# mynameisfiber/baton

Measured on NVIDIA H100. Metric: federated local samples/sec (whole box), ResNet-18 FedAvg, synthetic non-IID 32x32 shards, higher is better.
Workload: dtype bf16

## Files before the change

baton_b200/csrc/bindings.cpp:

```cpp
#include <ATen/cuda/CUDAContext.h>
#include <c10/cuda/CUDAGuard.h>
#include <torch/extension.h>

#include <optional>
#include <vector>

#include "launch.h"

namespace {

inline cudaStream_t cur_stream() { return at::cuda::getCurrentCUDAStream().stream(); }
inline void check(int rc, const char* what) {
  TORCH_CHECK(rc == 0, "baton_b200::", what, " failed with code ", rc,
              rc > 0 ? std::string(" (") + cudaGetErrorString(static_cast<cudaError_t>(rc)) + ")" : std::string());
}
inline const void* cptr(const at::Tensor& t) { return t.data_ptr(); }
inline void* ptr(at::Tensor& t) { return t.data_ptr(); }
template <class T>
inline T* opt_ptr(const std::optional<at::Tensor>& t) {
  return (t.has_value() && t->defined()) ? reinterpret_cast<T*>(t->data_ptr()) : nullptr;
}
#define CHECK_CUDA(x) TORCH_CHECK((x).is_cuda(), #x " must be a CUDA tensor")

inline const float* prox_anchor(const std::optional<at::Tensor>& anchor, int64_t numel, const at::Tensor& hyper) {
// ... 220 lines not shown
  return true;
}
bool conv_halo(const at::Tensor& src, const at::Tensor& w, at::Tensor out, int64_t stride, bool dgrad, int64_t mc,
               const std::optional<at::Tensor>& col_stats) {
  CHECK_CUDA(src); CHECK_CUDA(w); CHECK_CUDA(out);
  TORCH_CHECK(src.scalar_type() == at::kBFloat16 && w.scalar_type() == at::kBFloat16 && out.scalar_type() == at::kBFloat16 &&
              src.dim() == 4 && src.is_contiguous() && w.is_contiguous() && out.is_contiguous());
  TORCH_CHECK(stride == 1 || stride == 2, "conv_halo: stride 1 or 2");
  const int64_t c = src.size(3);
  const int64_t rows = src.size(0) * ((src.size(1) - 1) / stride + 1) * ((src.size(2) - 1) / stride + 1);
  TORCH_CHECK(rows > 0 && out.numel() % rows == 0, "conv_halo: out must hold [N*Ho*Wo, Nout] elements");
  const int64_t nout = out.numel() / rows;
  TORCH_CHECK(w.numel() == (dgrad ? c * 9 * nout : nout * 9 * c), "conv_halo: w must be [Cout, 9*Cin]");
  TORCH_CHECK(dgrad ? !col_stats.has_value()
                    : (!col_stats.has_value() || (col_stats->scalar_type() == at::kFloat && col_stats->numel() >= 2 * nout)),
              "conv_halo: col_stats is a [2 Cout] fp32 buffer of the forward");
  const c10::cuda::CUDAGuard guard(src.device());
  const int rc = b200_conv_halo(cptr(src), cptr(w), ptr(out), static_cast<int>(src.size(0)), static_cast<int>(src.size(1)),
                                static_cast<int>(src.size(2)), static_cast<int>(c), static_cast<int>(nout),
                                static_cast<int>(stride), dgrad ? 1 : 0, static_cast<int>(mc), opt_ptr<float>(col_stats),
                                cur_stream());
  if (rc == -2) return false;
  check(rc, "conv_halo");
  return true;
}
bool conv_igemm_dgrad_s2(const at::Tensor& dy, const at::Tensor& w, at::Tensor dx, int64_t kh, int64_t kw,
                         const std::vector<int64_t>& ntaps, const std::vector<int64_t>& taps, int64_t force_bn) {
  CHECK_CUDA(dy); CHECK_CUDA(w); CHECK_CUDA(dx);
  TORCH_CHECK(dy.scalar_type() == at::kBFloat16 && w.scalar_type() == at::kBFloat16 && dx.scalar_type() == at::kBFloat16 &&
              dy.dim() == 4 && dx.dim() == 4 && dy.is_contiguous() && w.is_contiguous() && dx.is_contiguous());
  TORCH_CHECK(ntaps.size() == 4 && taps.size() == 16, "conv_igemm_dgrad_s2: 4 classes x 4 taps");
  int nt[4], tw[16];
  for (int i = 0; i < 4; ++i) nt[i] = static_cast<int>(ntaps[i]);
  for (int i = 0; i < 16; ++i) tw[i] = static_cast<int>(taps[i]);
  const c10::cuda::CUDAGuard guard(dy.device());
  const int rc = b200_conv_igemm_dgrad_s2(cptr(dy), cptr(w), ptr(dx), static_cast<int>(dx.size(0)),
                                          static_cast<int>(dx.size(1)), static_cast<int>(dx.size(2)),
                                          static_cast<int>(dx.size(3)), static_cast<int>(dy.size(3)), static_cast<int>(kh),
                                          static_cast<int>(kw), static_cast<int>(dy.size(1)), static_cast<int>(dy.size(2)),
                                          nt, tw, static_cast<int>(force_bn), cur_stream());
  if (rc == -2) return false;
  check(rc, "conv_igemm_dgrad_s2");
  return true;
}
bool conv_igemm_wgrad(const at::Tensor& dy, const at::Tensor& x, at::Tensor dw, int64_t cout, int64_t kh, int64_t kw,
                      int64_t stride, int64_t pad, int64_t ho, int64_t wo, int64_t split_k, int64_t force_bn,
// ... 818 lines not shown
  const int in32 = pred.scalar_type() == at::kFloat;
  const int out32 = dpred.has_value() && dpred->defined() && dpred->scalar_type() == at::kFloat;
  check(b200_mse(pred.data_ptr(), in32, target.data_ptr<float>(), opt_ptr<void>(dpred), out32,
                 loss_acc.data_ptr<float>(), pred.numel(), static_cast<float>(grad_scale), cur_stream()),
        "mse");
}

}

PYBIND11_MODULE(TORCH_EXTENSION_NAME, m) {
  m.doc() = "baton_b200 sm_90a kernels";
  m.attr("MAX_RANKS") = B200_MAX_RANKS;
  m.def("gemm", &gemm);
  m.def("trace_set", &trace_set);
  m.def("attention_fwd", &attention_fwd);
  m.def("attention_bwd", &attention_bwd);
  m.def("bn_bwd_cluster", &bn_bwd_cluster);
  m.def("im2col_tma_probe", &im2col_tma_probe);
  m.def("conv_igemm_fwd", &conv_igemm_fwd);
  m.def("conv_igemm_wgrad", &conv_igemm_wgrad);
  m.def("conv_igemm_dgrad", &conv_igemm_dgrad);
  m.def("conv_igemm_dgrad_s2", &conv_igemm_dgrad_s2);
  m.def("conv_halo", &conv_halo);
  m.def("gemm_batched", &gemm_batched);
  m.def("gemm_fp8", &gemm_fp8);
  m.def("quant_mx_rows", &quant_mx_rows);
  m.def("quant_mx_cols", &quant_mx_cols);
  m.def("fused_sgd", &fused_sgd);
  m.def("fused_sgd_segments", &fused_sgd_segments);
  m.def("weighted_sum", &weighted_sum);
  m.def("fold_client", &fold_client);
  m.def("scaffold_corr", &scaffold_corr);
  m.def("scaffold_dc", &scaffold_dc);
  m.def("cast", &cast);
  m.def("gather_rows", &gather_rows);
  m.def("colsum", &colsum);
  m.def("add_bf16", &add_bf16);
  m.def("relu_bwd", &relu_bwd);
  m.def("gelu", &gelu);
  m.def("gelu_bwd", &gelu_bwd);
  m.def("pad_rows", &pad_rows);
  m.def("embedding_bwd", &embedding_bwd);
  m.def("fedavg_allreduce", &fedavg_allreduce);
  m.def("fedavg_allreduce_robust", &fedavg_allreduce_robust);
  m.def("fedavg_allreduce_krum", &fedavg_allreduce_krum);
  m.attr("KRUM_MAX_CTAS") = B200_KRUM_MAX_CTAS;
// ... 36 lines not shown
```

baton_b200/csrc/gemm_wgmma.cu:

```cuda
#define B200_TU_TAG 1
#include "ptx.cuh"
#include "epilogue.cuh"
#include "launch.h"
#include "pdl.cuh"
#include "sgd.cuh"

namespace b200 {

constexpr int BM = 128;
constexpr int BK = 64;
constexpr int WG_K = 16;
constexpr int GEMM_THREADS = 384;
constexpr int CONSUMER_WARPS = 8;
constexpr int CONSUMER_THREADS = 32 * CONSUMER_WARPS;
constexpr int MAX_STAGES = 8;
constexpr int S2_MAX_TAPS = 4;

struct GemmParams {
  int M, N, K;
  void* D;
  long long ldd;
  const float* bias;
  int out_fp32;
  int act;
// ... 339 lines not shown
  return w;
}
__device__ __forceinline__ int s2_dx_row(const GemmParams& p, int cls, int m) {
  if (m >= p.M) return -1;
  const int hw = p.conv_ho * p.conv_wo;
  const int n = m / hw, r = m - n * hw;
  const int i = r / p.conv_wo, j = r - i * p.conv_wo;
  const int h = 2 * i + (cls >> 1), w = 2 * j + (cls & 1);
  return (h < p.conv_h && w < p.conv_w) ? (n * p.conv_h + h) * p.conv_w + w : -1;
}
template <int BN>
__device__ __forceinline__ void s2_load_ktile(const CUtensorMap* tmA, const CUtensorMap* tmB, const GemmParams& p,
                                              uint8_t* sa, uint8_t* sb, uint64_t* bar, int cls, int kt, int m0, int n0) {
  const int cblocks = p.conv_cin >> 6;
  const int slot = kt / cblocks, cb = kt - slot * cblocks;
  const int tw = s2_tap(p, cls, slot);
  const int q0 = m0 % p.conv_wo, t0 = m0 / p.conv_wo;
  tma_load_im2col_4d(sa, tmA, bar, cb * 64, q0, t0 % p.conv_ho, t0 / p.conv_ho, (tw >> 24) & 0xff, (tw >> 16) & 0xff);
  const int wcol = (tw & 0xffff) * p.conv_ncol + n0;
#pragma unroll
  for (int j = 0; j < BN / 64; ++j) tma_load_2d(sb + j * 8192, tmB, bar, wcol + j * 64, cb * 64);
}

template <int BN, int STAGES, int CONV = 0, bool SGD = false, bool AFFINE = false, bool PROX = false, bool SCAF = false,
          bool ADAM = false>
__global__ void __launch_bounds__(GEMM_THREADS, 1)
gemm_bf16_fixed_kernel(const __grid_constant__ CUtensorMap tmA, const __grid_constant__ CUtensorMap tmB,
                         const GemmParams p) {
  using L = SmemLayout<BN>;
  static_assert(STAGES * L::STAGE_BYTES >= L::PART_BYTES, "the drained ring must hold the fp32 accumulator tile");
  extern __shared__ __align__(1024) uint8_t smem_raw[];
  uint8_t* smem = reinterpret_cast<uint8_t*>((reinterpret_cast<uintptr_t>(smem_raw) + 1023) & ~uintptr_t(1023));
  uint64_t* full_bar = reinterpret_cast<uint64_t*>(smem + STAGES * L::STAGE_BYTES);
  uint64_t* empty_bar = full_bar + STAGES;
  float* cstat = reinterpret_cast<float*>(empty_bar + STAGES);

  griddep_launch_dependents();
  const int warp = threadIdx.x >> 5;
  int m0 = blockIdx.y * BM;
  const int cls = CONV == 4 ? s2_class(p, m0) : 0;
  const int n0 = blockIdx.x * BN;
  const int k_tiles_total = CONV == 4 ? s2_ntaps(p, cls) * (p.conv_cin >> 6) : (p.K + BK - 1) / BK;
  const int bz_outer = p.batched ? static_cast<int>(blockIdx.z) / p.batch_inner : 0;
  const int bz_inner = p.batched ? static_cast<int>(blockIdx.z) % p.batch_inner : 0;
  const int kt_begin = p.batched ? 0 : blockIdx.z * p.k_tiles_per_split;
  int kt_end = kt_begin + p.k_tiles_per_split;
  if (kt_end > k_tiles_total) kt_end = k_tiles_total;
  const int num_kt = kt_end - kt_begin;

  if (warp == 0 && elect_one()) {
    tma_prefetch_desc(&tmA);
    tma_prefetch_desc(&tmB);
    for (int s = 0; s < STAGES; ++s) {
      mbar_init(&full_bar[s], 1);
      mbar_init(&empty_bar[s], CONSUMER_WARPS);
    }
    fence_barrier_init();
  }
  __syncthreads();
  griddep_wait();

  if (warp == 0) {
    if (elect_one()) {
      if (p.tile_flags != nullptr) {
        const int rows_here = (p.N - n0) < BN ? (p.N - n0) : BN;
        const uint32_t need = p.flag_epoch_ptr != nullptr ? *reinterpret_cast<const volatile uint32_t*>(p.flag_epoch_ptr)
                                                          : p.flag_epoch;
        wait_arrival_flags(p.tile_flags, p.flag_elem_off + static_cast<long long>(n0) * p.ldb,
                           p.flag_elem_off + static_cast<long long>(n0 + rows_here) * p.ldb - 1, p.flag_tile_elems, need);
        if (p.flag_bias_off >= 0)
          wait_arrival_flags(p.tile_flags, p.flag_bias_off + n0, p.flag_bias_off + n0 + rows_here - 1,
                             p.flag_tile_elems, need);
        fence_proxy_async_all();
      }
      TRACE_POINT();
      for (int i = 0; i < num_kt; ++i) {
        const int s = i % STAGES;
        const uint32_t ph = (i / STAGES) & 1;
        mbar_wait(&empty_bar[s], ph ^ 1);
        uint8_t* sa = smem + s * L::STAGE_BYTES;
        uint8_t* sb = sa + L::A_BYTES;
        const int k0 = (kt_begin + i) * BK;
        if constexpr (CONV == 2) {
          const int live = (p.N - n0 + 63) / 64 < BN / 64 ? (p.N - n0 + 63) / 64 : BN / 64;
          mbar_expect_tx(&full_bar[s], L::A_BYTES + live * 8192);
        } else {
          mbar_expect_tx(&full_bar[s], L::STAGE_BYTES);
        }
        if (p.batched) {
          if (!p.a_mn) {
            tma_load_4d(sa, &tmA, &full_bar[s], k0, m0, bz_inner, bz_outer);
          } else {
#pragma unroll
            for (int j = 0; j < BM / 64; ++j)
              tma_load_4d(sa + j * 8192, &tmA, &full_bar[s], m0 + j * 64, k0, bz_inner, bz_outer);
          }
          if (!p.b_mn) {
            tma_load_4d(sb, &tmB, &full_bar[s], k0, n0, bz_inner, bz_outer);
          } else {
#pragma unroll
            for (int j = 0; j < BN / 64; ++j)
              tma_load_4d(sb + j * 8192, &tmB, &full_bar[s], n0 + j * 64, k0, bz_inner, bz_outer);
          }
        } else if constexpr (CONV == 4) {
          s2_load_ktile<BN>(&tmA, &tmB, p, sa, sb, &full_bar[s], cls, kt_begin + i, m0, n0);
        } else {
        if constexpr (CONV == 1 || CONV == 3) {
          const int kt = kt_begin + i;
          const int cblocks = p.conv_cin >> 6;
          const int tap = kt / cblocks, cb = kt - tap * cblocks;
          const int fr = tap / p.conv_kw, fs = tap - fr * p.conv_kw;
          const int q0 = m0 % p.conv_wo, t0 = m0 / p.conv_wo;
          tma_load_im2col_4d(sa, &tmA, &full_bar[s], cb * 64, q0 * p.conv_stride - p.conv_pad,
                             (t0 % p.conv_ho) * p.conv_stride - p.conv_pad, t0 / p.conv_ho, fs, fr);
        } else if (!p.a_mn) {
          tma_load_2d(sa, &tmA, &full_bar[s], k0, m0);
        } else {
#pragma unroll
          for (int j = 0; j < BM / 64; ++j)
            tma_load_2d(sa + j * 8192, &tmA, &full_bar[s], m0 + j * 64, k0);
        }
        if constexpr (CONV == 2) {
          const int q0 = k0 % p.conv_wo, t0 = k0 / p.conv_wo;
          const int w0 = q0 * p.conv_stride - p.conv_pad, h0 = (t0 % p.conv_ho) * p.conv_stride - p.conv_pad;
          const int img = t0 / p.conv_ho;
#pragma unroll
          for (int j = 0; j < BN / 64; ++j) {
            const int col = n0 + j * 64;
// ... 96 lines not shown
        } else {
          _Pragma("unroll") for (int j = 0; j < 32; ++j) if (col0 + j < p.N) d[j] = v[j];
        }
      } else {
        __nv_bfloat16* d = reinterpret_cast<__nv_bfloat16*>(drow) + col0;
        if (full && vec_ok) {
#pragma unroll
          for (int j = 0; j < 32; j += 8) {
            uint4 o;
            o.x = pack_bf16x2(v[j], v[j + 1]);
            o.y = pack_bf16x2(v[j + 2], v[j + 3]);
            o.z = pack_bf16x2(v[j + 4], v[j + 5]);
            o.w = pack_bf16x2(v[j + 6], v[j + 7]);
            *reinterpret_cast<uint4*>(d + j) = o;
          }
        } else {
          _Pragma("unroll") for (int j = 0; j < 32; ++j) if (col0 + j < p.N) d[j] = __float2bfloat16_rn(v[j]);
        }
      }
    }
    if (threadIdx.x == 128) TRACE_POINT();
    if (want_stats) {
      named_bar_sync(1, CONSUMER_THREADS);
      for (int i = threadIdx.x - 128; i < 2 * BN; i += CONSUMER_THREADS) {
        const int col = i < BN ? i : i - BN;
        if (n0 + col < p.N)
          atomicAdd(p.col_stats + (i < BN ? 0 : p.N) + n0 + col,
                    cstat[i] + cstat[2 * BN + i] + cstat[4 * BN + i] + cstat[6 * BN + i]);
      }
    }
  }
}


constexpr int EPI_PITCH = 144;
constexpr int EPI_WARP_BYTES = 32 * EPI_PITCH;

template <int BN>
__device__ __forceinline__ void epilogue_tile(const GemmParams& p, const float* acc_tile, int q, int half, int m0,
                                              int n0, uint8_t* stage, bool vec_ok, size_t d_off = 0) {
  using L = SmemLayout<BN>;
  const int lane = static_cast<int>(lane_id());
  const int row = m0 + q * 32 + lane;
  const float* arow = acc_tile + (q * 32 + lane) * L::PART_PITCH;
  const int elt = p.out_fp32 ? 4 : 2;
  const bool fast = vec_ok && !p.atomic_out && (p.N % 8 == 0);
  if (!fast) {
#pragma unroll 1
    for (int c = half * 32; c < BN; c += 64) {
      uint32_t r[32];
      acc_ld_row32(arow + c, r);
// ... 151 lines not shown
    }
  }
}


template <int BN, bool CLUSTER, int CONV = 0, bool AFFINE = false>
__global__ void __launch_bounds__(GEMM_THREADS, 1)
gemm_bf16_splitk_kernel(const __grid_constant__ CUtensorMap tmA, const __grid_constant__ CUtensorMap tmB,
                        const GemmParams p) {
  using L = SmemLayout<BN>;
  extern __shared__ __align__(1024) uint8_t smem_raw[];
  uint8_t* smem = reinterpret_cast<uint8_t*>((reinterpret_cast<uintptr_t>(smem_raw) + 1023) & ~uintptr_t(1023));
  const int STAGES = p.stages;
  const int ring_bytes = STAGES * L::STAGE_BYTES;
  const int data_bytes = L::PART_BYTES > ring_bytes ? L::PART_BYTES : ring_bytes;
  uint64_t* full_bar = reinterpret_cast<uint64_t*>(smem + data_bytes);
  uint64_t* empty_bar = full_bar + MAX_STAGES;
  float* cstat = reinterpret_cast<float*>(empty_bar + MAX_STAGES);

  griddep_launch_dependents();
  const int warp = threadIdx.x >> 5;
  const int m0 = blockIdx.y * BM;
  const int n0 = blockIdx.x * BN;
  const int k_tiles_total = (p.K + BK - 1) / BK;
  const int kt_begin = blockIdx.z * p.k_tiles_per_split;
  int kt_end = kt_begin + p.k_tiles_per_split;
  if (kt_end > k_tiles_total) kt_end = k_tiles_total;
  const int num_kt = kt_end - kt_begin;

  if (warp == 0 && elect_one()) {
    tma_prefetch_desc(&tmA);
    tma_prefetch_desc(&tmB);
    for (int s = 0; s < STAGES; ++s) {
      mbar_init(&full_bar[s], 1);
      mbar_init(&empty_bar[s], CONSUMER_WARPS);
    }
    fence_barrier_init();
  }
  __syncthreads();
  griddep_wait();

  if (warp == 0) {
    if (elect_one()) {
      if (p.tile_flags != nullptr) {
        const int rows_here = (p.N - n0) < BN ? (p.N - n0) : BN;
        const uint32_t need = p.flag_epoch_ptr != nullptr ? *reinterpret_cast<const volatile uint32_t*>(p.flag_epoch_ptr)
                                                          : p.flag_epoch;
        wait_arrival_flags(p.tile_flags, p.flag_elem_off + static_cast<long long>(n0) * p.ldb,
                           p.flag_elem_off + static_cast<long long>(n0 + rows_here) * p.ldb - 1, p.flag_tile_elems, need);
        if (p.flag_bias_off >= 0)
          wait_arrival_flags(p.tile_flags, p.flag_bias_off + n0, p.flag_bias_off + n0 + rows_here - 1,
                             p.flag_tile_elems, need);
        fence_proxy_async_all();
      }
      int s = 0;
      uint32_t ph = 0;
      for (int i = 0; i < num_kt; ++i) {
        mbar_wait(&empty_bar[s], ph ^ 1);
        uint8_t* sa = smem + s * L::STAGE_BYTES;
        uint8_t* sb = sa + L::A_BYTES;
        const int k0 = (kt_begin + i) * BK;
        mbar_expect_tx(&full_bar[s], L::STAGE_BYTES);
        if constexpr (CONV == 1 || CONV == 3) {
          const int kt = kt_begin + i;
          const int cblocks = p.conv_cin >> 6;
          const int tap = kt / cblocks, cb = kt - tap * cblocks;
          const int fr = tap / p.conv_kw, fs = tap - fr * p.conv_kw;
          const int q0 = m0 % p.conv_wo, t0 = m0 / p.conv_wo;
          tma_load_im2col_4d(sa, &tmA, &full_bar[s], cb * 64, q0 * p.conv_stride - p.conv_pad,
                             (t0 % p.conv_ho) * p.conv_stride - p.conv_pad, t0 / p.conv_ho, fs, fr);
        } else if (!p.a_mn) {
          tma_load_2d(sa, &tmA, &full_bar[s], k0, m0);
        } else {
#pragma unroll
          for (int j = 0; j < BM / 64; ++j)
            tma_load_2d(sa + j * 8192, &tmA, &full_bar[s], m0 + j * 64, k0);
        }
        if constexpr (CONV == 3) {
          const int kt = kt_begin + i;
          const int cblocks = p.conv_cin >> 6;
          const int tap = kt / cblocks, cb = kt - tap * cblocks;
          const int wcol = (p.conv_taps - 1 - tap) * p.conv_ncol + n0;
#pragma unroll
          for (int j = 0; j < BN / 64; ++j) tma_load_2d(sb + j * 8192, &tmB, &full_bar[s], wcol + j * 64, cb * 64);
        } else if (!p.b_mn) {
          tma_load_2d(sb, &tmB, &full_bar[s], k0, n0);
        } else {
#pragma unroll
          for (int j = 0; j < BN / 64; ++j) tma_load_2d(sb + j * 8192, &tmB, &full_bar[s], n0 + j * 64, k0);
        }
        if (++s == STAGES) { s = 0; ph ^= 1; }
      }
    }
  } else if (warp >= 4) {
    const int ew = warp - 4;
    float acc[BN / 2];
    int s = 0;
    uint32_t ph = 0;
    consume_ktiles<BN>(acc, smem, STAGES, full_bar, empty_bar, s, ph, num_kt, p.a_mn, p.b_mn, ew >> 2);
    named_bar_sync(1, CONSUMER_THREADS);
    float* part = reinterpret_cast<float*>(smem);
// ... 52 lines not shown
            cq[j] = fmaf(rnd, rnd, cq[j]);
          }
        }
        if (row < p.M && col0 < p.N) store_row_chunk<8, AFFINE>(p, row, col0, v, vec_ok);
      }
      if (want_stats) {
#pragma unroll
        for (int j = 0; j < 8; ++j) {
#pragma unroll
          for (int o = CG; o < 32; o <<= 1) {
            cs[j] += __shfl_xor_sync(0xffffffffu, cs[j], o);
            cq[j] += __shfl_xor_sync(0xffffffffu, cq[j], o);
          }
        }
        const int wq = t >> 5, ln = t & 31;
        if (ln < CG) {
#pragma unroll
          for (int j = 0; j < 8; ++j) {
            cstat[wq * 2 * BN + ln * 8 + j] = cs[j];
            cstat[wq * 2 * BN + BN + ln * 8 + j] = cq[j];
          }
        }
        named_bar_sync(2, 128);
        for (int i = t; i < 2 * BN; i += 128) {
          const int col = i < BN ? i : i - BN;
          if (n0 + col < p.N) {
            const float v = cstat[i] + cstat[2 * BN + i] + cstat[4 * BN + i] + cstat[6 * BN + i];
            atomicAdd(p.col_stats + (i < BN ? 0 : p.N) + n0 + col, v);
          }
        }
      }
    }
    cluster_sync_all();
  }
}


typedef CUresult (*EncodeTiledFn)(CUtensorMap*, CUtensorMapDataType, cuuint32_t, void*, const cuuint64_t*,
                                  const cuuint64_t*, const cuuint32_t*, const cuuint32_t*, CUtensorMapInterleave,
                                  CUtensorMapSwizzle, CUtensorMapL2promotion, CUtensorMapFloatOOBfill);

static EncodeTiledFn get_encode_fn() {
  static thread_local bool ctx_bound = false;
  if (!ctx_bound) {
    cudaFree(nullptr);
    ctx_bound = true;
  }
  static EncodeTiledFn fn = nullptr;
  if (fn == nullptr) {
    void* ptr = nullptr;
    cudaDriverEntryPointQueryResult qres;
// ... 443 lines not shown
  }
  if (max_taps == 0) return -2;
  const int bn = clamp_bn(force_bn > 0 ? force_bn : (Cin > 64 ? 128 : 64));
  CUtensorMap ta, tb;
  int rc = b200_encode_map_im2col_bf16(&ta, dy, N, Ho, Wo, Cout, 1, 1, 1, 0, 64, BM);
  if (rc) return rc;
  rc = make_map(&tb, w, Cout, static_cast<long long>(KH) * KW * Cin, static_cast<long long>(KH) * KW * Cin, 64, BK);
  if (rc) return rc;
  const int k_tiles = max_taps * (Cout / 64);
  p.M = static_cast<int>(M); p.N = Cin; p.K = k_tiles * BK; p.D = dx; p.ldd = Cin; p.bias = nullptr; p.out_fp32 = 0;
  p.act = 0; p.a_mn = 0; p.b_mn = 1; p.k_tiles_per_split = k_tiles; p.cluster_k = 1; p.atomic_out = 0;
  p.col_stats = nullptr;
  p.tile_flags = nullptr; p.flag_epoch = 0; p.alpha = 1.0f; p.flag_elem_off = 0; p.flag_tile_elems = 0;
  p.ldb = static_cast<long long>(KH) * KW * Cin;
  p.flag_bias_off = -1; p.flag_epoch_ptr = nullptr;
  p.batched = 0; p.batch_inner = 1; p.batch_count = 1; p.d_outer = 0; p.d_inner = 0;
  p.conv_ho = Ho; p.conv_wo = Wo; p.conv_stride = 2; p.conv_pad = 0; p.conv_kw = KW; p.conv_cin = Cout;
  p.conv_taps = KH * KW; p.conv_ncol = Cin; p.conv_h = H; p.conv_w = W;
  dim3 grid((Cin + bn - 1) / bn, static_cast<unsigned>(4 * tiles_m), 1);
  if (bn == 128) return launch_fixed<128, 6, 4>(ta, tb, p, grid, stream);
  return launch_fixed<64, 8, 4>(ta, tb, p, grid, stream);
}

extern "C" int b200_conv_igemm_wgrad(const void* dy, const void* x, float* dw, int N, int H, int W, int Cin, int Cout,
                                     int KH, int KW, int stride, int pad, int Ho, int Wo, int split_k, int force_bn,
                                     const B200SgdEpilogue* sgd, cudaStream_t stream) {
  using namespace b200;
  const long long Mp = static_cast<long long>(N) * Ho * Wo;
  const int Kc = KH * KW * Cin;
  if (Mp <= 0 || Cout <= 0) return 0;
  if (Cin % 64 != 0 || Cout % 8 != 0 || Mp > (1ll << 30) || (reinterpret_cast<uintptr_t>(x) & 15) ||
      (reinterpret_cast<uintptr_t>(dy) & 15) || (reinterpret_cast<uintptr_t>(dw) & 15))
    return -2;
  const int bn = clamp_bn(force_bn > 0 ? force_bn : (Kc > 64 ? 128 : 64));
  CUtensorMap ta, tb;
  int rc = make_map(&ta, dy, Mp, Cout, Cout, 64, BK);
  if (rc) return rc;
  rc = b200_encode_map_im2col_bf16(&tb, x, N, H, W, Cin, KH, KW, stride, pad, 64, 64);
  if (rc) return rc;
  const int k_tiles = static_cast<int>((Mp + BK - 1) / BK);
  if (split_k < 1) split_k = 1;
  if (split_k > k_tiles) split_k = k_tiles;
  const int per = (k_tiles + split_k - 1) / split_k;
  split_k = (k_tiles + per - 1) / per;
  if (sgd != nullptr && split_k != 1) return B200_SGD_EPILOGUE_DECLINED;
  GemmParams p;
// ... 21 lines not shown
```

baton_b200/csrc/launch.h:

```cpp
#pragma once
#include <cuda_runtime.h>
#include <stdint.h>

#define B200_MAX_RANKS 16

extern "C" {

struct B200SgdEpilogue {
  float* theta;
  void* theta_bf16;
  float* mom;
  const float* hyper;
  int nesterov;
  const float* anchor;
  const float* corr;
  float* v;
};
#define B200_SGD_EPILOGUE_DECLINED (-6)

struct B200AffineEpilogue {
  const float* scale;
  const float* shift;
  const void* residual;
  long long ldr;
// ... 1 lines not shown
};
#define B200_AFFINE_EPILOGUE_DECLINED (-7)

int b200_gemm_bf16(const void* a, const void* b, void* d, const float* bias, int M, int N, int K, long long lda,
                   long long ldb, long long ldd, int a_mn, int b_mn, int out_fp32, int act, int split_k, int accumulate,
                   float alpha, const uint32_t* tile_flags, uint32_t flag_epoch, long long flag_elem_off, int flag_tile_elems,
                   long long flag_bias_off, int force_bn, float* col_stats, const uint32_t* flag_epoch_ptr,
                   const B200SgdEpilogue* sgd, const B200AffineEpilogue* affine, cudaStream_t stream);
int b200_gemm_bf16_batched(const void* a, const void* b, void* d, int M, int N, int K, long long lda, long long ldb,
                           long long ldd, int a_mn, int b_mn, int out_fp32, int act, float alpha, int n_outer,
                           int n_inner, long long a_outer, long long a_inner, long long b_outer, long long b_inner,
                           long long d_outer, long long d_inner, int accumulate, cudaStream_t stream);
int b200_attention_fwd(const void* qkv, void* out, void* probs, int B, int S, int H, int dh, float scale,
                       cudaStream_t stream);
int b200_attention_bwd(const void* qkv, const void* dout, const void* probs, void* dqkv, int B, int S, int H, int dh,
                       float scale, cudaStream_t stream);
int b200_conv_igemm_fwd(const void* x, const void* w, void* y, int N, int H, int W, int Cin, int Cout, int KH, int KW,
                        int stride, int pad, int Ho, int Wo, int cluster_k, int force_bn, float* col_stats,
                        const B200AffineEpilogue* affine, cudaStream_t stream);
int b200_conv_igemm_dgrad(const void* dy, const void* w, void* dx, int N, int H, int W, int Cin, int Cout, int KH, int KW,
                          int pad, int Ho, int Wo, int cluster_k, int force_bn, cudaStream_t stream);
int b200_conv_igemm_dgrad_s2(const void* dy, const void* w, void* dx, int N, int H, int W, int Cin, int Cout, int KH,
                             int KW, int Ho, int Wo, const int* ntaps, const int* taps, int force_bn, cudaStream_t stream);
int b200_conv_igemm_wgrad(const void* dy, const void* x, float* dw, int N, int H, int W, int Cin, int Cout, int KH, int KW,
                          int stride, int pad, int Ho, int Wo, int split_k, int force_bn, const B200SgdEpilogue* sgd,
                          cudaStream_t stream);
int b200_conv_halo(const void* src, const void* w, void* out, int N, int H, int W, int C, int Nout, int stride,
                   int dgrad, int mc, float* col_stats, cudaStream_t stream);
int b200_im2col_tma_probe(const void* x, void* col, int N, int H, int W, int C, int KH, int KW, int stride, int pad,
                          int Ho, int Wo, cudaStream_t stream);
int b200_gemm_fp8(const void* a, const void* b, void* d, const float* bias, const void* sfa, const void* sfb, int M, int N,
                  int K, long long lda, long long ldb, long long ldd, int out_fp32, int act, int split_k, int accumulate,
                  float alpha, cudaStream_t stream);
int b200_quant_mx_rows(const void* x, void* q, void* sf, long long R, int C, long long ld_in, int Cp, cudaStream_t stream);
int b200_quant_mx_cols(const void* x, void* q, void* sf, long long R, int C, long long ld_in, long long Rp,
                       cudaStream_t stream);
int b200_gemm_simt(const void* a, const void* b, void* d, const float* bias, int M, int N, int K, long long lda,
                   long long ldb, long long ldd, int a_mn, int b_mn, int out_fp32, int act, int accumulate,
                   float alpha, cudaStream_t stream);

int b200_fused_sgd(float* w, float* g, float* mom, void* w_bf16, long long n, const float* hyper, int zero_grad,
                   int nesterov, const unsigned long long* wire_slot, const float* pack_global,
                   const float* pack_scale, long long n_pack, int wire_fp32, const float* prox_anchor,
                   const float* corr, float* adam_v, cudaStream_t stream);
int b200_fused_sgd_segments(float* w, float* g, float* mom, void* w_bf16, const long long* segments, int n_seg,
                            const float* hyper, int nesterov, const float* prox_anchor, const float* corr,
// ... 180 lines not shown
```

baton_b200/ops/functional.py:

```python
from __future__ import annotations

import collections
import functools
from typing import List, Optional, Sequence, Tuple

import torch

from ._ext import load

BF16 = torch.bfloat16
NUM_SMS = 132


def _pitch(t: torch.Tensor) -> int:
    assert t.dim() == 2 and (t.stride(1) == 1 or t.shape[1] == 1), "GEMM operand must have unit inner stride"
    return t.stride(0) if t.shape[0] > 1 else max(t.stride(0), t.shape[1])


def _tma_ok(t: torch.Tensor) -> bool:
    return t.dtype == BF16 and _pitch(t) % 8 == 0 and t.data_ptr() % 16 == 0


def pick_bn(M: int, N: int) -> int:
    m_tiles = (M + 127) // 128
# ... 352 lines not shown


def halo_smem_bytes(h: int, w: int, c: int = 64, stride: int = 1) -> int:
    ho, wo = conv_out_size(h, 3, stride, 1), conv_out_size(w, 3, stride, 1)
    box = (HALO_BM // (ho * wo)) * (stride * (ho - 1) + 3) * (stride * (wo - 1) + 3) * 128
    k_tiles = 9 * (c // 64)
    return c // 64 * round_up(box, 1024) + k_tiles * 8192 + round_up(1 + k_tiles, 16) * 8 + 4 * 64 * 4 + 1024


def halo_eligible(kh: int, kw: int, stride: int, pad: int, c: int, h: int, w: int,
                  affine: Optional[dict] = None, dgrad: bool = False) -> bool:
    if kh != 3 or kw != 3 or pad != 1 or (stride, c) not in _HALO_FORMS or (dgrad and stride != 1):
        return False
    hw = conv_out_size(h, 3, stride, 1) * conv_out_size(w, 3, stride, 1)
    return (hw <= HALO_BM and HALO_BM % hw == 0 and affine is None and
            halo_smem_bytes(h, w, c, stride) <= _HALO_MAX_SMEM)


def halo_cluster(m_rows: int) -> int:
    tiles = (m_rows + HALO_BM - 1) // HALO_BM
    return 4 if tiles % 4 == 0 else 2 if tiles % 2 == 0 else 1


def _conv_path(path: Optional[str], eligible: bool) -> str:
    if path is None:
        return "halo" if eligible else "im2col"
    if path not in ("halo", "im2col"):
        raise ValueError("path must be None, 'halo' or 'im2col', not {!r}".format(path))
    if path == "halo" and not eligible:
        raise ValueError("the halo kernel does not take this convolution (see halo_eligible)")
    return path


def conv_igemm_fwd(x: torch.Tensor, w2d: torch.Tensor, kh: int, kw: int, stride: int, pad: int,
                   col_stats: Optional[torch.Tensor] = None, affine: Optional[dict] = None,
                   cluster_k: Optional[int] = None, force_bn: int = 0,
                   out: Optional[torch.Tensor] = None, path: Optional[str] = None,
                   mc: Optional[int] = None) -> Optional[torch.Tensor]:
    n, h, w, c = x.shape
    cout = w2d.shape[0]
    if c % 64 or w2d.shape[1] != kh * kw * c or not x.is_contiguous() or not w2d.is_contiguous():
        return None
    ho, wo = conv_out_size(h, kh, stride, pad), conv_out_size(w, kw, stride, pad)
    M, K = n * ho * wo, kh * kw * c
    halo = halo_eligible(kh, kw, stride, pad, c, h, w, affine) and cout % 8 == 0
    if _conv_path(path, halo) == "halo":
        y = out if out is not None else torch.empty((M, cout), dtype=BF16, device=x.device)
        if not load().conv_halo(x, w2d, y, stride, False, mc or halo_cluster(M), col_stats):
            raise RuntimeError("conv_halo declined a convolution halo_eligible admits")
        return y
    bn = force_bn or pick_bn(M, cout)
    if cluster_k is None:
        cluster_k = pick_cluster_k(M, cout, K, bn)
    y = out if out is not None else torch.empty((M, cout), dtype=BF16, device=x.device)
    af = affine or {}
    ok = load().conv_igemm_fwd(x, w2d, y, kh, kw, stride, pad, ho, wo, cluster_k, bn, col_stats, af.get("scale"),
                               af.get("shift"), af.get("residual"), bool(af.get("relu", False)))
    return y if ok else None


S2_MAX_TAPS = 4


def conv_s2_dgrad_taps(kh: int, kw: int, pad: int, ho: int, wo: int) -> Optional[List[List[Tuple[int, int, int]]]]:
    classes = []
    for a in (0, 1):
        for b in (0, 1):
            taps = []
            for r in range(kh):
                if (a + pad - r) % 2:
                    continue
                dp = (a + pad - r) // 2
                for s in range(kw):
                    if (b + pad - s) % 2:
                        continue
                    dq = (b + pad - s) // 2
                    if dp < 0 or dq < 0:
                        return None
                    if dp < ho and dq < wo:
                        taps.append((r * kw + s, dp, dq))
            if len(taps) > S2_MAX_TAPS:
                return None
            classes.append(taps)
    return classes


def conv_igemm_dgrad(dy: torch.Tensor, w2d: torch.Tensor, in_shape, kh: int, kw: int, pad: int, stride: int = 1,
                     out: Optional[torch.Tensor] = None, path: Optional[str] = None,
                     mc: Optional[int] = None, cluster_k: Optional[int] = None) -> Optional[torch.Tensor]:
    n, h, w, c = in_shape
    cout = dy.shape[-1]
    if c % 64 or cout % 64 or w2d.shape[1] != kh * kw * c or not dy.is_contiguous() or not w2d.is_contiguous():
        return None
    if _conv_path(path, halo_eligible(kh, kw, stride, pad, cout, h, w, dgrad=True)) == "halo":
        dx = out if out is not None else torch.empty((n, h, w, c), dtype=BF16, device=dy.device)
        if not load().conv_halo(dy, w2d, dx, 1, True, mc or halo_cluster(n * h * w), None):
            raise RuntimeError("conv_halo declined a convolution halo_eligible admits")
        return dx
    if stride == 1:
        M, K = n * h * w, kh * kw * cout
        bn = pick_bn(M, c)
        dx = out if out is not None else torch.empty((n, h, w, c), dtype=BF16, device=dy.device)
        if cluster_k is None:
            cluster_k = pick_cluster_k(M, c, K, bn)
        ok = load().conv_igemm_dgrad(dy, w2d, dx, kh, kw, pad, cluster_k, bn)
        return dx if ok else None
    if stride != 2:
        return None
    ho, wo = dy.shape[1], dy.shape[2]
    classes = conv_s2_dgrad_taps(kh, kw, pad, ho, wo)
    if classes is None:
        return None
    bn = pick_bn(4 * n * ho * wo, c)
    words = [[t | dp << 16 | dq << 24 for t, dp, dq in taps] + [0] * (S2_MAX_TAPS - len(taps)) for taps in classes]
    dx = out if out is not None else torch.empty((n, h, w, c), dtype=BF16, device=dy.device)
    ok = load().conv_igemm_dgrad_s2(dy, w2d, dx, kh, kw, [len(t) for t in classes], [x for ws in words for x in ws], bn)
    return dx if ok else None


def conv_igemm_wgrad_(dy2d: torch.Tensor, x: torch.Tensor, dw2d: torch.Tensor, kh: int, kw: int, stride: int,
# ... 173 lines not shown
```

Baseline: 225,500.

## Add per-image GEMM conv path that skips padded taps for tiny feature maps

Adds a new conv mode (CONV==5) that treats each image as a GEMM row and walks only the kernel taps that land inside the image. This skips the zero-padding work im2col does on very small maps (ho*wo<=4, as in late ResNet-18 layers on 32x32 inputs). It covers forward with column stats and dgrad, uses a split-K cluster, and is chosen automatically when the skipped fraction is at least half. The cost is more index arithmetic per k-tile, a small grid with M=N images, and a fixed BN of 64.

```diff
diff --git a/baton_b200/csrc/bindings.cpp b/baton_b200/csrc/bindings.cpp
--- a/baton_b200/csrc/bindings.cpp
+++ b/baton_b200/csrc/bindings.cpp
@@ -266,6 +266,30 @@
                                 cur_stream());
   if (rc == -2) return false;
   check(rc, "conv_halo");
+  return true;
+}
+bool conv_image(const at::Tensor& src, const at::Tensor& w, at::Tensor out, int64_t kh, int64_t kw, int64_t stride,
+                int64_t pad, bool dgrad, int64_t cluster_k, const std::optional<at::Tensor>& col_stats) {
+  CHECK_CUDA(src); CHECK_CUDA(w); CHECK_CUDA(out);
+  TORCH_CHECK(src.scalar_type() == at::kBFloat16 && w.scalar_type() == at::kBFloat16 && out.scalar_type() == at::kBFloat16 &&
+              src.dim() == 4 && out.dim() == 4 && src.is_contiguous() && w.is_contiguous() && out.is_contiguous() &&
+              w.dim() == 2 && src.size(0) == out.size(0));
+  const at::Tensor& x = dgrad ? out : src;
+  const at::Tensor& y = dgrad ? src : out;
+  const int64_t cin = x.size(3), cout = y.size(3);
+  TORCH_CHECK(stride > 0 && pad >= 0 && y.size(1) == (x.size(1) + 2 * pad - kh) / stride + 1 &&
+              y.size(2) == (x.size(2) + 2 * pad - kw) / stride + 1, "conv_image: output map does not match the convolution");
+  TORCH_CHECK(w.size(0) == cout && w.size(1) == kh * kw * cin, "conv_image: w must be [Cout, kh*kw*Cin]");
+  TORCH_CHECK(!col_stats.has_value() || (!dgrad && col_stats->scalar_type() == at::kFloat && col_stats->numel() >= 2 * cout),
+              "conv_image: col_stats is a [2 Cout] fp32 buffer of the forward");
+  const c10::cuda::CUDAGuard guard(src.device());
+  const int rc = b200_conv_image(cptr(src), cptr(w), ptr(out), static_cast<int>(x.size(0)), static_cast<int>(x.size(1)),
+                                 static_cast<int>(x.size(2)), static_cast<int>(cin), static_cast<int>(cout),
+                                 static_cast<int>(kh), static_cast<int>(kw), static_cast<int>(stride),
+                                 static_cast<int>(pad), dgrad ? 1 : 0, static_cast<int>(cluster_k),
+                                 opt_ptr<float>(col_stats), cur_stream());
+  if (rc == -2) return false;
+  check(rc, "conv_image");
   return true;
 }
 bool conv_igemm_dgrad_s2(const at::Tensor& dy, const at::Tensor& w, at::Tensor dx, int64_t kh, int64_t kw,
@@ -1130,6 +1154,7 @@
   m.def("conv_igemm_dgrad", &conv_igemm_dgrad);
   m.def("conv_igemm_dgrad_s2", &conv_igemm_dgrad_s2);
   m.def("conv_halo", &conv_halo);
+  m.def("conv_image", &conv_image);
   m.def("gemm_batched", &gemm_batched);
   m.def("gemm_fp8", &gemm_fp8);
   m.def("quant_mx_rows", &quant_mx_rows);
diff --git a/baton_b200/csrc/gemm_wgmma.cu b/baton_b200/csrc/gemm_wgmma.cu
--- a/baton_b200/csrc/gemm_wgmma.cu
+++ b/baton_b200/csrc/gemm_wgmma.cu
@@ -385,6 +385,88 @@
   for (int j = 0; j < BN / 64; ++j) tma_load_2d(sb + j * 8192, tmB, bar, wcol + j * 64, cb * 64);
 }
 
+struct ImgDim {
+  int first, step, n;
+};
+__device__ __forceinline__ ImgDim img_dim(const GemmParams& p, int q, int k, int in, int out) {
+  ImgDim d;
+  if (!p.b_mn) {
+    const int i0 = q * p.conv_stride - p.conv_pad;
+    const int lo = i0 < 0 ? -i0 : 0, hi = in - i0 < k ? in - i0 : k;
+    d.first = lo; d.step = 1; d.n = hi > lo ? hi - lo : 0;
+  } else {
+    const int t = q + p.conv_pad, st = p.conv_stride;
+    int lo = t - st * (out - 1);
+    lo = lo < 0 ? 0 : lo;
+    lo += (t - lo) % st;
+    const int hi = t < k - 1 ? t : k - 1;
+    d.n = hi >= lo ? (hi - lo) / st + 1 : 0;
+    d.first = st == 1 ? hi : lo; d.step = st == 1 ? -1 : st;
+  }
+  return d;
+}
+__device__ __forceinline__ int img_cols(const GemmParams& p) {
+  return p.b_mn ? p.conv_ncol : p.N / (p.conv_ho * p.conv_wo);
+}
+__device__ __forceinline__ int img_tile(const GemmParams& p, int n0, ImgDim& dr, ImgDim& dc) {
+  const int ow = p.b_mn ? p.conv_w : p.conv_wo;
+  const int pix = n0 / img_cols(p), oh = pix / ow, oc = pix - oh * ow;
+  dr = img_dim(p, oh, p.conv_taps / p.conv_kw, p.conv_h, p.conv_ho);
+  dc = img_dim(p, oc, p.conv_kw, p.conv_w, p.conv_wo);
+  return pix;
+}
+__device__ __forceinline__ int img_ktiles(const GemmParams& p, int n0) {
+  ImgDim dr, dc;
+  img_tile(p, n0, dr, dc);
+  return dr.n * dc.n * (p.conv_cin >> 6);
+}
+struct ImgWalk {
+  int a0, a_r, a_s, b0, b_r, b_s, c0, ns, jr, js, cb;
+};
+__device__ __forceinline__ ImgWalk img_walk(const GemmParams& p, int n0, int kt) {
+  ImgDim dr, dc;
+  const int pix = img_tile(p, n0, dr, dc);
+  const int ow = p.b_mn ? p.conv_w : p.conv_wo;
+  const int oh = pix / ow, oc = pix - oh * ow;
+  int gh0, gw0, dgh, dgw, gwidth;
+  if (!p.b_mn) {
+    gh0 = oh * p.conv_stride - p.conv_pad + dr.first; gw0 = oc * p.conv_stride - p.conv_pad + dc.first;
+    dgh = dr.step; dgw = dc.step; gwidth = p.conv_w;
+  } else {
+    gh0 = (oh + p.conv_pad - dr.first) / p.conv_stride; gw0 = (oc + p.conv_pad - dc.first) / p.conv_stride;
+    dgh = p.conv_stride == 1 ? 1 : -1; dgw = dgh; gwidth = p.conv_wo;
+  }
+  ImgWalk w;
+  w.a0 = (gh0 * gwidth + gw0) * p.conv_cin; w.a_r = dgh * gwidth * p.conv_cin; w.a_s = dgw * p.conv_cin;
+  w.b0 = (dr.first * p.conv_kw + dc.first) * p.conv_ncol; w.b_r = dr.step * p.conv_kw * p.conv_ncol;
+  w.b_s = dc.step * p.conv_ncol;
+  w.c0 = n0 - pix * img_cols(p);
+  w.ns = dc.n;
+  const int cblocks = p.conv_cin >> 6;
+  const int j = kt / cblocks;
+  w.cb = kt - j * cblocks;
+  w.jr = dc.n > 0 ? j / dc.n : 0;
+  w.js = j - w.jr * dc.n;
+  return w;
+}
+template <int BN>
+__device__ __forceinline__ void img_load_ktile(const CUtensorMap* tmA, const CUtensorMap* tmB, const GemmParams& p,
+                                               uint8_t* sa, uint8_t* sb, uint64_t* bar, int m0, ImgWalk& w) {
+  const int a = w.a0 + w.jr * w.a_r + w.js * w.a_s + w.cb * 64;
+  const int b = w.b0 + w.jr * w.b_r + w.js * w.b_s;
+  tma_load_2d(sa, tmA, bar, a, m0);
+  if (!p.b_mn) {
+    tma_load_2d(sb, tmB, bar, b + w.cb * 64, w.c0);
+  } else {
+#pragma unroll
+    for (int jj = 0; jj < BN / 64; ++jj) tma_load_2d(sb + jj * 8192, tmB, bar, b + w.c0 + jj * 64, w.cb * 64);
+  }
+  if (++w.cb == (p.conv_cin >> 6)) {
+    w.cb = 0;
+    if (++w.js == w.ns) { w.js = 0; ++w.jr; }
+  }
+}
+
 template <int BN, int STAGES, int CONV = 0, bool SGD = false, bool AFFINE = false, bool PROX = false, bool SCAF = false,
           bool ADAM = false>
 __global__ void __launch_bounds__(GEMM_THREADS, 1)
@@ -403,7 +485,9 @@
   int m0 = blockIdx.y * BM;
   const int cls = CONV == 4 ? s2_class(p, m0) : 0;
   const int n0 = blockIdx.x * BN;
-  const int k_tiles_total = CONV == 4 ? s2_ntaps(p, cls) * (p.conv_cin >> 6) : (p.K + BK - 1) / BK;
+  const int k_tiles_total = CONV == 4   ? s2_ntaps(p, cls) * (p.conv_cin >> 6)
+                            : CONV == 5 ? img_ktiles(p, n0)
+                                        : (p.K + BK - 1) / BK;
   const int bz_outer = p.batched ? static_cast<int>(blockIdx.z) / p.batch_inner : 0;
   const int bz_inner = p.batched ? static_cast<int>(blockIdx.z) % p.batch_inner : 0;
   const int kt_begin = p.batched ? 0 : blockIdx.z * p.k_tiles_per_split;
@@ -437,6 +521,8 @@
         fence_proxy_async_all();
       }
       TRACE_POINT();
+      ImgWalk walk{};
+      if constexpr (CONV == 5) walk = img_walk(p, n0, kt_begin);
       for (int i = 0; i < num_kt; ++i) {
         const int s = i % STAGES;
         const uint32_t ph = (i / STAGES) & 1;
@@ -467,6 +553,8 @@
           }
         } else if constexpr (CONV == 4) {
           s2_load_ktile<BN>(&tmA, &tmB, p, sa, sb, &full_bar[s], cls, kt_begin + i, m0, n0);
+        } else if constexpr (CONV == 5) {
+          img_load_ktile<BN>(&tmA, &tmB, p, sa, sb, &full_bar[s], m0, walk);
         } else {
         if constexpr (CONV == 1 || CONV == 3) {
           const int kt = kt_begin + i;
@@ -609,11 +697,17 @@
     if (threadIdx.x == 128) TRACE_POINT();
     if (want_stats) {
       named_bar_sync(1, CONSUMER_THREADS);
+      const int st_n = CONV == 5 ? img_cols(p) : p.N, st_c0 = CONV == 5 ? n0 % st_n : n0;
       for (int i = threadIdx.x - 128; i < 2 * BN; i += CONSUMER_THREADS) {
         const int col = i < BN ? i : i - BN;
-        if (n0 + col < p.N)
+        if constexpr (CONV == 5) {
+          if (n0 + col < p.N)
+            atomicAdd(p.col_stats + (i < BN ? 0 : st_n) + st_c0 + col,
+                      cstat[i] + cstat[2 * BN + i] + cstat[4 * BN + i] + cstat[6 * BN + i]);
+        } else if (n0 + col < p.N) {
           atomicAdd(p.col_stats + (i < BN ? 0 : p.N) + n0 + col,
                     cstat[i] + cstat[2 * BN + i] + cstat[4 * BN + i] + cstat[6 * BN + i]);
+        }
       }
     }
   }
@@ -811,11 +905,12 @@
   const int warp = threadIdx.x >> 5;
   const int m0 = blockIdx.y * BM;
   const int n0 = blockIdx.x * BN;
-  const int k_tiles_total = (p.K + BK - 1) / BK;
-  const int kt_begin = blockIdx.z * p.k_tiles_per_split;
-  int kt_end = kt_begin + p.k_tiles_per_split;
+  const int k_tiles_total = CONV == 5 ? img_ktiles(p, n0) : (p.K + BK - 1) / BK;
+  const int per = CONV == 5 ? (k_tiles_total + p.cluster_k - 1) / p.cluster_k : p.k_tiles_per_split;
+  const int kt_begin = blockIdx.z * per;
+  int kt_end = kt_begin + per;
   if (kt_end > k_tiles_total) kt_end = k_tiles_total;
-  const int num_kt = kt_end - kt_begin;
+  const int num_kt = CONV == 5 && kt_end < kt_begin ? 0 : kt_end - kt_begin;
 
   if (warp == 0 && elect_one()) {
     tma_prefetch_desc(&tmA);
@@ -844,13 +939,17 @@
       }
       int s = 0;
       uint32_t ph = 0;
+      ImgWalk walk{};
+      if constexpr (CONV == 5) walk = img_walk(p, n0, kt_begin);
       for (int i = 0; i < num_kt; ++i) {
         mbar_wait(&empty_bar[s], ph ^ 1);
         uint8_t* sa = smem + s * L::STAGE_BYTES;
         uint8_t* sb = sa + L::A_BYTES;
         const int k0 = (kt_begin + i) * BK;
         mbar_expect_tx(&full_bar[s], L::STAGE_BYTES);
-        if constexpr (CONV == 1 || CONV == 3) {
+        if constexpr (CONV == 5) {
+          img_load_ktile<BN>(&tmA, &tmB, p, sa, sb, &full_bar[s], m0, walk);
+        } else if constexpr (CONV == 1 || CONV == 3) {
           const int kt = kt_begin + i;
           const int cblocks = p.conv_cin >> 6;
           const int tap = kt / cblocks, cb = kt - tap * cblocks;
@@ -865,7 +964,8 @@
           for (int j = 0; j < BM / 64; ++j)
             tma_load_2d(sa + j * 8192, &tmA, &full_bar[s], m0 + j * 64, k0);
         }
-        if constexpr (CONV == 3) {
+        if constexpr (CONV == 5) {
+        } else if constexpr (CONV == 3) {
           const int kt = kt_begin + i;
           const int cblocks = p.conv_cin >> 6;
           const int tap = kt / cblocks, cb = kt - tap * cblocks;
@@ -964,11 +1064,13 @@
           }
         }
         named_bar_sync(2, 128);
+        const int st_n = CONV == 5 ? img_cols(p) : p.N, st_c0 = CONV == 5 ? n0 % st_n : n0;
         for (int i = t; i < 2 * BN; i += 128) {
           const int col = i < BN ? i : i - BN;
           if (n0 + col < p.N) {
             const float v = cstat[i] + cstat[2 * BN + i] + cstat[4 * BN + i] + cstat[6 * BN + i];
-            atomicAdd(p.col_stats + (i < BN ? 0 : p.N) + n0 + col, v);
+            if constexpr (CONV == 5) atomicAdd(p.col_stats + (i < BN ? 0 : st_n) + st_c0 + col, v);
+            else atomicAdd(p.col_stats + (i < BN ? 0 : p.N) + n0 + col, v);
           }
         }
       }
@@ -1458,6 +1560,45 @@
   return launch_fixed<64, 8, 4>(ta, tb, p, grid, stream);
 }
 
+extern "C" int b200_conv_image(const void* src, const void* w, void* out, int N, int H, int W, int Cin, int Cout, int KH,
+                               int KW, int stride, int pad, int dgrad, int cluster_k, float* col_stats,
+                               cudaStream_t stream) {
+  using namespace b200;
+  const int Ho = (H + 2 * pad - KH) / stride + 1, Wo = (W + 2 * pad - KW) / stride + 1;
+  if (N <= 0) return 0;
+  const long long src_cols = dgrad ? static_cast<long long>(Ho) * Wo * Cout : static_cast<long long>(H) * W * Cin;
+  const long long out_cols = dgrad ? static_cast<long long>(H) * W * Cin : static_cast<long long>(Ho) * Wo * Cout;
+  if (Cin % 64 != 0 || Cout % 64 != 0 || Ho <= 0 || Wo <= 0 || stride <= 0 || pad < 0 || out_cols > (1ll << 30) ||
+      (dgrad && col_stats != nullptr) || (reinterpret_cast<uintptr_t>(src) & 15) ||
+      (reinterpret_cast<uintptr_t>(w) & 15) || (reinterpret_cast<uintptr_t>(out) & 15))
+    return -2;
+  if (cluster_k != 1 && cluster_k != 2 && cluster_k != 4 && cluster_k != 8) return -5;
+  constexpr int bn = 64;
+  const int gathered = dgrad ? Cout : Cin;
+  CUtensorMap ta, tb;
+  int rc = make_map(&ta, src, N, src_cols, src_cols, BK, BM);
+  if (rc) return rc;
+  const long long wk = static_cast<long long>(KH) * KW * Cin;
+  rc = dgrad ? make_map(&tb, w, Cout, wk, wk, 64, BK) : make_map(&tb, w, Cout, wk, wk, BK, bn);
+  if (rc) return rc;
+  const int max_kt = KH * KW * (gathered / 64);
+  while (cluster_k > 1 && (cluster_k - 1) * ((max_kt + cluster_k - 1) / cluster_k) >= max_kt) cluster_k >>= 1;
+  const int per = (max_kt + cluster_k - 1) / cluster_k;
+  GemmParams p;
+  p.M = N; p.N = static_cast<int>(out_cols); p.K = max_kt * BK; p.D = out; p.ldd = out_cols; p.bias = nullptr;
+  p.out_fp32 = 0; p.act = 0; p.a_mn = 0; p.b_mn = dgrad ? 1 : 0; p.k_tiles_per_split = per; p.cluster_k = cluster_k;
+  p.atomic_out = 0; p.col_stats = col_stats;
+  p.tile_flags = nullptr; p.flag_epoch = 0; p.alpha = 1.0f; p.flag_elem_off = 0; p.flag_tile_elems = 0; p.ldb = wk;
+  p.flag_bias_off = -1; p.flag_epoch_ptr = nullptr;
+  p.batched = 0; p.batch_inner = 1; p.batch_count = 1; p.d_outer = 0; p.d_inner = 0;
+  p.stages = per < 8 ? (per < 2 ? 2 : per) : 8;
+  p.conv_h = H; p.conv_w = W; p.conv_ho = Ho; p.conv_wo = Wo; p.conv_stride = stride; p.conv_pad = pad;
+  p.conv_kw = KW; p.conv_taps = KH * KW; p.conv_cin = gathered; p.conv_ncol = Cin;
+  dim3 grid(static_cast<unsigned>(out_cols / bn), static_cast<unsigned>((N + BM - 1) / BM), cluster_k);
+  if (cluster_k > 1) return launch_cfg<bn, 5>(ta, tb, p, grid, stream);
+  return launch_fixed<bn, 8, 5>(ta, tb, p, grid, stream);
+}
+
 extern "C" int b200_conv_igemm_wgrad(const void* dy, const void* x, float* dw, int N, int H, int W, int Cin, int Cout,
                                      int KH, int KW, int stride, int pad, int Ho, int Wo, int split_k, int force_bn,
                                      const B200SgdEpilogue* sgd, cudaStream_t stream) {
diff --git a/baton_b200/csrc/launch.h b/baton_b200/csrc/launch.h
--- a/baton_b200/csrc/launch.h
+++ b/baton_b200/csrc/launch.h
@@ -47,6 +47,8 @@
                           int pad, int Ho, int Wo, int cluster_k, int force_bn, cudaStream_t stream);
 int b200_conv_igemm_dgrad_s2(const void* dy, const void* w, void* dx, int N, int H, int W, int Cin, int Cout, int KH,
                              int KW, int Ho, int Wo, const int* ntaps, const int* taps, int force_bn, cudaStream_t stream);
+int b200_conv_image(const void* src, const void* w, void* out, int N, int H, int W, int Cin, int Cout, int KH, int KW,
+                    int stride, int pad, int dgrad, int cluster_k, float* col_stats, cudaStream_t stream);
 int b200_conv_igemm_wgrad(const void* dy, const void* x, float* dw, int N, int H, int W, int Cin, int Cout, int KH, int KW,
                           int stride, int pad, int Ho, int Wo, int split_k, int force_bn, const B200SgdEpilogue* sgd,
                           cudaStream_t stream);
diff --git a/baton_b200/ops/functional.py b/baton_b200/ops/functional.py
--- a/baton_b200/ops/functional.py
+++ b/baton_b200/ops/functional.py
@@ -398,13 +398,35 @@
     return 4 if tiles % 4 == 0 else 2 if tiles % 2 == 0 else 1
 
 
-def _conv_path(path: Optional[str], eligible: bool) -> str:
+IMAGE_MAX_PIXELS = 4
+
+
+def image_gemm_eligible(kh: int, kw: int, stride: int, pad: int, c: int, cout: int, h: int, w: int,
+                        affine: Optional[dict] = None) -> bool:
+    ho, wo = conv_out_size(h, kh, stride, pad), conv_out_size(w, kw, stride, pad)
+    return (c % 64 == 0 and cout % 64 == 0 and ho >= 1 and wo >= 1 and ho * wo <= IMAGE_MAX_PIXELS and h * w > 1 and
+            affine is None)
+
+
+def image_gemm_pays(kh: int, kw: int, stride: int, pad: int, h: int, w: int) -> bool:
+    ho, wo = conv_out_size(h, kh, stride, pad), conv_out_size(w, kw, stride, pad)
+    rows = sum(1 for p in range(ho) for r in range(kh) if 0 <= p * stride - pad + r < h)
+    cols = sum(1 for q in range(wo) for s in range(kw) if 0 <= q * stride - pad + s < w)
+    return 2 * rows * cols <= ho * wo * kh * kw
+
+
+IMAGE_CLUSTER = 4
+
+
+def _conv_path(path: Optional[str], eligible: bool, image: bool = False, pays: bool = True) -> str:
     if path is None:
-        return "halo" if eligible else "im2col"
-    if path not in ("halo", "im2col"):
-        raise ValueError("path must be None, 'halo' or 'im2col', not {!r}".format(path))
+        return "halo" if eligible else "image" if image and pays else "im2col"
+    if path not in ("halo", "image", "im2col"):
+        raise ValueError("path must be None, 'halo', 'image' or 'im2col', not {!r}".format(path))
     if path == "halo" and not eligible:
         raise ValueError("the halo kernel does not take this convolution (see halo_eligible)")
+    if path == "image" and not image:
+        raise ValueError("the per-image GEMM does not take this convolution (see image_gemm_eligible)")
     return path
 
 
@@ -420,10 +442,18 @@
     ho, wo = conv_out_size(h, kh, stride, pad), conv_out_size(w, kw, stride, pad)
     M, K = n * ho * wo, kh * kw * c
     halo = halo_eligible(kh, kw, stride, pad, c, h, w, affine) and cout % 8 == 0
-    if _conv_path(path, halo) == "halo":
+    kind = _conv_path(path, halo, image_gemm_eligible(kh, kw, stride, pad, c, cout, h, w, affine),
+                      image_gemm_pays(kh, kw, stride, pad, h, w))
+    if kind == "halo":
         y = out if out is not None else torch.empty((M, cout), dtype=BF16, device=x.device)
         if not load().conv_halo(x, w2d, y, stride, False, mc or halo_cluster(M), col_stats):
             raise RuntimeError("conv_halo declined a convolution halo_eligible admits")
+        return y
+    if kind == "image":
+        y = out if out is not None else torch.empty((M, cout), dtype=BF16, device=x.device)
+        ck = cluster_k or IMAGE_CLUSTER
+        if not load().conv_image(x, w2d, y.view(n, ho, wo, cout), kh, kw, stride, pad, False, ck, col_stats):
+            raise RuntimeError("conv_image declined a convolution image_gemm_eligible admits")
         return y
     bn = force_bn or pick_bn(M, cout)
     if cluster_k is None:
@@ -468,10 +498,18 @@
     cout = dy.shape[-1]
     if c % 64 or cout % 64 or w2d.shape[1] != kh * kw * c or not dy.is_contiguous() or not w2d.is_contiguous():
         return None
-    if _conv_path(path, halo_eligible(kh, kw, stride, pad, cout, h, w, dgrad=True)) == "halo":
+    kind = _conv_path(path, halo_eligible(kh, kw, stride, pad, cout, h, w, dgrad=True),
+                      image_gemm_eligible(kh, kw, stride, pad, c, cout, h, w), image_gemm_pays(kh, kw, stride, pad, h, w))
+    if kind == "halo":
         dx = out if out is not None else torch.empty((n, h, w, c), dtype=BF16, device=dy.device)
         if not load().conv_halo(dy, w2d, dx, 1, True, mc or halo_cluster(n * h * w), None):
             raise RuntimeError("conv_halo declined a convolution halo_eligible admits")
+        return dx
+    if kind == "image":
+        dx = out if out is not None else torch.empty((n, h, w, c), dtype=BF16, device=dy.device)
+        ck = cluster_k or IMAGE_CLUSTER
+        if not load().conv_image(dy, w2d, dx, kh, kw, stride, pad, True, ck, None):
+            raise RuntimeError("conv_image declined a convolution image_gemm_eligible admits")
         return dx
     if stride == 1:
         M, K = n * h * w, kh * kw * cout
```

After: 227,000 (median of 6 runs). Within noise of the previous version (+0.7%).
